# kotaro-kinoshita/yomitoku

Hardware: NVIDIA H100
Metric: pages/sec (DBNet->PARSeq OCR, synthetic 1600x1200 pages, ~200 crops/page) (higher is better)
Workload: dtype f16

## Files before the change

yomitoku_b200/csrc/gemm_tc.cu:

```cuda
#include "gemm_tc.h"

#include <cstdarg>
#include <cstdlib>
#include <cstdio>
#include <cstring>
#include <atomic>
#include <mutex>
#include <vector>

#include "ptx.cuh"

namespace ytk {

static thread_local char g_err[512] = "";
void set_error(const char* fmt, ...) {
    va_list ap;
    va_start(ap, fmt);
    vsnprintf(g_err, sizeof(g_err), fmt, ap);
    va_end(ap);
}
const char* last_error() { return g_err; }

static std::atomic<long long> g_launches{0};
void count_launch(int n) { g_launches.fetch_add(n, std::memory_order_relaxed); }
long long launch_count() { return g_launches.load(std::memory_order_relaxed); }

int pdl_launch_attr(cudaLaunchAttribute* attr) {
    static const bool on = getenv("YTK_PDL") != nullptr && getenv("YTK_NO_PDL") == nullptr;
    if (!on) return 0;
    attr[0].id = cudaLaunchAttributeProgrammaticStreamSerialization;
    attr[0].val.programmaticStreamSerializationAllowed = 1;
    return 1;
}

bool first_launch_on_device(unsigned long long* mask) {
    int d = 0;
    cudaGetDevice(&d);
    const unsigned long long bit = 1ull << (d & 63);
    if (*mask & bit) return false;
    *mask |= bit;
    return true;
}

int num_sms() {
    static int n = 0;
    if (n == 0) {
        int dev = 0;
        cudaGetDevice(&dev);
        cudaDeviceGetAttribute(&n, cudaDevAttrMultiProcessorCount, dev);
        if (n <= 0) n = 132;
    }
    return n;
}

constexpr int kBlockM = 128;
constexpr int kBlockK = 64;
constexpr int kABytes = kBlockM * kBlockK * 2;
constexpr int kThreads = 384;
constexpr int kProducerWarp = 8;
constexpr int kStagePitch = 80;
constexpr int kEpiStageBytes = 8 * 32 * kStagePitch;
constexpr int kAccPitch = 68;
constexpr int kAccBytes = 2 * 64 * kAccPitch * 4;

constexpr int kEpiBufBytes = 32 * 64;
constexpr int epi_tma_nbuf(int ) { return 2; }
constexpr int kSmemLimit = 232448;
constexpr int kSmemFixed = 1024  + 1024  + 512 ;

template <int BLOCK_N, int EPI_BYTES = kEpiStageBytes>
struct TileCfg {
    static constexpr int kBBytes = BLOCK_N * kBlockK * 2;
    static constexpr int kStageBytes = kABytes + kBBytes;
    static constexpr int kRingBudget = kSmemLimit - kSmemFixed - kAccBytes - EPI_BYTES;
    static constexpr int kStages = (kRingBudget / kStageBytes) > 8 ? 8 : (kRingBudget / kStageBytes);
    static constexpr int kRingBytes = kStages * kStageBytes;
    static constexpr int kSmemBytes = kRingBytes + kAccBytes + EPI_BYTES + kSmemFixed;
    static_assert(kStages >= 3, "K pipeline depth");
    static_assert(kSmemBytes <= kSmemLimit, "shared memory budget");
    static_assert((kRingBytes + kAccBytes) % 2048 == 0, "epilogue buffers must stay 2 KB aligned");
};

__device__ __noinline__ void copy_elems(void* dst, const void* src, int n, int esz) {
    if (esz == 4)
        for (int e = 0; e < n; ++e) reinterpret_cast<uint32_t*>(dst)[e] = reinterpret_cast<const uint32_t*>(src)[e];
    else
        for (int e = 0; e < n; ++e) reinterpret_cast<uint16_t*>(dst)[e] = reinterpret_cast<const uint16_t*>(src)[e];
}
__device__ __forceinline__ float gelu_fast(float x) {
    const float t = fminf(fabsf(x), 5.7f);
    float p = fmaf(4.278742836e-06f, t, -1.279820572e-05f);
    p = fmaf(p, t, -5.757861654e-04f);
    p = fmaf(p, t, 7.670783438e-03f);
    p = fmaf(p, t, -5.294856429e-02f);
    p = fmaf(p, t, -4.590439200e-01f);
    p = fmaf(p, t, -1.151126981e+00f);
    const float a = __fmul_rn(p, t);
    float e;
    asm("ex2.approx.ftz.f32 %0, %1;" : "=f"(e) : "f"(a));
    return fmaf(__fmul_rn(t, -0.5f), e, fmaxf(x, 0.f));
}
__device__ __forceinline__ void gelu_fast2(float& x0, float& x1) {
    x0 = gelu_fast(x0);
    x1 = gelu_fast(x1);
}

struct TileCoord {
    int img, h0, w0, n0;
};
__device__ __forceinline__ TileCoord decode_tile(const GemmArgs& a, int tile, int block_n) {
    TileCoord t;
    int m_tile = tile / a.tiles_n;
    int n_tile = tile - m_tile * a.tiles_n;
    int tw = m_tile % a.tiles_w;
    int t2 = m_tile / a.tiles_w;
    int th = t2 % a.tiles_h;
    t.img = t2 / a.tiles_h;
    t.h0 = th * (kBlockM >> a.bw_log2);
    t.w0 = tw << a.bw_log2;
    t.n0 = n_tile * block_n;
    return t;
}

template <int BLOCK_N, int RESID, int DIRECT>
using KernelCfg = TileCfg<BLOCK_N, DIRECT == 2 ? 8 * epi_tma_nbuf(RESID) * kEpiBufBytes : kEpiStageBytes>;

template <int BLOCK_N, int OUT_F32, int RESID, int MODE, int DIRECT>
__global__ void __launch_bounds__(kThreads, 1) gemm_tc_kernel(const __grid_constant__ GemmMaps maps,
                                                              const __grid_constant__ GemmArgs args) {
    using Cfg = KernelCfg<BLOCK_N, RESID, DIRECT>;
    constexpr int kEpiBytes = Cfg::kSmemBytes - Cfg::kRingBytes - kAccBytes - kSmemFixed;
    constexpr int stage_bytes = Cfg::kStageBytes;
    constexpr int nstages = Cfg::kStages;
    extern __shared__ uint8_t smem_raw[];
    const uint32_t raw_addr = smem_u32(smem_raw);
    uint8_t* smem = smem_raw + ((1024u - (raw_addr & 1023u)) & 1023u);
    const int worker = static_cast<int>(blockIdx.x);
    const int n_workers = static_cast<int>(gridDim.x);

    float* acc_smem = reinterpret_cast<float*>(smem + Cfg::kRingBytes);
    uint8_t* epi_stage = smem + Cfg::kRingBytes + kAccBytes;
    float* fin_w = reinterpret_cast<float*>(epi_stage + kEpiBytes);
    uint64_t* full_bar = reinterpret_cast<uint64_t*>(epi_stage + kEpiBytes + 1024);
    uint64_t* empty_bar = full_bar + 8;
    [[maybe_unused]] uint64_t* rbar_base = empty_bar + 8;

    const int warp = threadIdx.x >> 5;
    const int lane = threadIdx.x & 31;

    if (threadIdx.x == 0) {
        for (int i = 0; i < nstages; ++i) {
            mbar_init(&full_bar[i], 1);
            mbar_init(&empty_bar[i], 8);
        }
        if constexpr (DIRECT == 2 && RESID != 0) {
            for (int i = 0; i < 32; ++i) mbar_init(&rbar_base[i], 1);
        }
        fence_mbar_init();
        tma_prefetch_desc(&maps.a[0]);
        tma_prefetch_desc(&maps.b);
        if constexpr (DIRECT == 2) {
            tma_prefetch_desc(&maps.out);
            if constexpr (RESID != 0) {
                tma_prefetch_desc(&maps.resid);
                tma_prefetch_desc(&maps.resid_pf);
            }
        }
    }
    if constexpr (MODE == EPI_CONVT_FINAL) {
        if (threadIdx.x < 256) fin_w[threadIdx.x] = args.fin_w[threadIdx.x];
    }
    __syncthreads();
    pdl_wait();
    pdl_launch_dependents();

    const int tiles_m = args.n_img * args.tiles_h * args.tiles_w;
    const int num_kb = args.ntaps * args.kpt;
    const int total_units = tiles_m * args.tiles_n;

    if (warp >= kProducerWarp) {
        setmaxnreg_dec<40>();
        if (warp == kProducerWarp && lane == 0) {
            int stage = 0;
            uint32_t phase = 0;
            [[maybe_unused]] auto prefetch_resid = [&](int u2) {
                if (u2 >= total_units) return;
                const TileCoord c2 = decode_tile(args, u2, BLOCK_N);
                tma_prefetch_l2_4d(&maps.resid_pf, c2.n0, c2.w0, c2.h0, c2.img);
            };
            if constexpr (DIRECT == 2 && RESID != 0) {
                if (args.epi_pf) prefetch_resid(worker);
            }
            for (int u = worker; u < total_units; u += n_workers) {
                const TileCoord tc = decode_tile(args, u, BLOCK_N);
                if constexpr (DIRECT == 2 && RESID != 0) {
                    if (args.epi_pf) prefetch_resid(u + n_workers);
                }
                int tap = 0, cb = 0;
                for (int kb = 0; kb < num_kb; ++kb) {
                    mbar_wait(&empty_bar[stage], phase ^ 1u);
                    uint8_t* sa = smem + stage * stage_bytes;
                    uint8_t* sb = sa + kABytes;
                    const ConvTap tp = args.taps[tap];
                    mbar_expect_tx(&full_bar[stage], Cfg::kStageBytes);
                    tma_load_4d(sa, &maps.a[tp.map], &full_bar[stage], cb * kBlockK, tc.w0 + tp.dw, tc.h0 + tp.dh,
                                tc.img);
                    tma_load_4d(sb, &maps.b, &full_bar[stage], kb * kBlockK, tc.n0, 0, 0);
                    if (++cb == args.kpt) {
                        cb = 0;
                        ++tap;
                    }
                    if (++stage == nstages) {
                        stage = 0;
                        phase ^= 1u;
                    }
                }
            }
        }
    } else {
        setmaxnreg_inc<232>();
        const int wg = warp >> 2, wl = warp & 3;
        const int q = 2 * wg + (wl & 1);
        const int wset = wl >> 1;
        float* acc_buf = acc_smem + wg * 64 * kAccPitch;
        const float* my_acc = acc_buf + ((wl & 1) * 32 + lane) * kAccPitch;
        float acc[BLOCK_N / 2];
#pragma unroll
        for (int i = 0; i < BLOCK_N / 2; ++i) acc[i] = 0.f;
        int ring_stage = 0;
        uint32_t ring_phase = 0;
        auto mma_tile = [&]() {
            const uint32_t a_off = static_cast<uint32_t>(wg * 64 * 128);
            int prev = -1;
            for (int kb = 0; kb < num_kb; ++kb) {
                mbar_wait(&full_bar[ring_stage], ring_phase);
                const uint32_t a_addr = smem_u32(smem + ring_stage * stage_bytes);
                const uint64_t da = wgmma_desc_sw128(a_addr + a_off);
                const uint64_t db = wgmma_desc_sw128(a_addr + kABytes);
                reg_fence(acc);
                wgmma_fence();
#pragma unroll
                for (int k = 0; k < kBlockK / 16; ++k)
                    wgmma_ss<BLOCK_N>(acc, da + static_cast<uint64_t>(2 * k), db + static_cast<uint64_t>(2 * k),
                                      (kb | k) != 0 ? 1u : 0u);
                wgmma_commit();
                wgmma_wait<1>();
                reg_fence(acc);
                if (prev >= 0) {
                    __syncwarp();
                    if (lane == 0) mbar_arrive(&empty_bar[prev]);
                }
                prev = ring_stage;
                if (++ring_stage == nstages) {
                    ring_stage = 0;
                    ring_phase ^= 1u;
                }
            }
            wgmma_wait<0>();
            reg_fence(acc);
            __syncwarp();
            if (lane == 0) mbar_arrive(&empty_bar[prev]);
        };
        auto dump_slice = [&](int s) {
            named_bar_sync(1 + wg, 128);
            const int r0 = wl * 16 + (lane >> 2), c2 = (lane & 3) * 2;
#pragma unroll
            for (int j = 0; j < BLOCK_N / 8; ++j) {
                if ((j >> 3) == s) {
                    float* p = acc_buf + r0 * kAccPitch + (j & 7) * 8 + c2;
                    *reinterpret_cast<float2*>(p) = make_float2(acc[4 * j], acc[4 * j + 1]);
                    *reinterpret_cast<float2*>(p + 8 * kAccPitch) = make_float2(acc[4 * j + 2], acc[4 * j + 3]);
                }
            }
            named_bar_sync(1 + wg, 128);
        };
        auto load_chunk = [&](int c, float (&f)[32]) {
            const float4* a4 = reinterpret_cast<const float4*>(my_acc + (c & 1) * 32);
#pragma unroll
            for (int j = 0; j < 8; ++j) {
                const float4 x = a4[j];
                f[4 * j + 0] = x.x;
                f[4 * j + 1] = x.y;
                f[4 * j + 2] = x.z;
                f[4 * j + 3] = x.w;
            }
        };
        if constexpr (DIRECT == 2) {
            static_assert(MODE == EPI_NORMAL, "TMA epilogue: plain stores only");
            static_assert(RESID == 0 || (RESID == 2) == (OUT_F32 != 0), "TMA epilogue: residual and output boxes match");
            constexpr int NBUF = epi_tma_nbuf(RESID);
            constexpr int LOOK = NBUF - 1;
            constexpr int CPP = OUT_F32 ? 16 : 32;
            constexpr int NPASS = 32 / CPP;
            const int bw_mask = (1 << args.bw_log2) - 1;
            const int qw = (q * 32) & bw_mask;
            const int qh = (q * 32) >> args.bw_log2;
            uint8_t* bufs = epi_stage + warp * (NBUF * kEpiBufBytes);
            [[maybe_unused]] uint64_t* rbar = rbar_base + warp * 4;
            const int sw = args.epi_swz ? ((lane >> 1) & 3) : 0;
            const int row_off = lane * 64;
            [[maybe_unused]] int pf_u = worker, pf_c = wset, pf_p = 0, pf_g = 0;
            [[maybe_unused]] TileCoord pf_tc{};
            [[maybe_unused]] auto pf_seek = [&]() {
                while (pf_u < total_units) {
                    pf_tc = decode_tile(args, pf_u, BLOCK_N);
                    if (pf_c < BLOCK_N / 32 && pf_tc.n0 + pf_c * 32 + pf_p * CPP < args.Cout) return;
                    pf_c = wset;
                    pf_p = 0;
                    pf_u += n_workers;
                }
            };
            [[maybe_unused]] auto pf_step = [&]() {
                if (++pf_p == NPASS) {
                    pf_p = 0;
                    pf_c += 2;
                }
                pf_seek();
            };
            [[maybe_unused]] auto pf_issue = [&]() {
                const int b = pf_g % NBUF;
                mbar_expect_tx(&rbar[b], kEpiBufBytes);
                tma_load_4d(bufs + b * kEpiBufBytes, &maps.resid, &rbar[b], pf_tc.n0 + pf_c * 32 + pf_p * CPP,
                            pf_tc.w0 + qw, pf_tc.h0 + qh, pf_tc.img);
                ++pf_g;
            };
            if constexpr (RESID != 0) {
                if (lane == 0) {
                    pf_seek();
                    for (int k = 0; k < LOOK && pf_u < total_units; ++k) {
                        pf_issue();
                        pf_step();
                    }
                }
            }
            int gc = 0;
            for (int u = worker; u < total_units; u += n_workers) {
                const TileCoord tc = decode_tile(args, u, BLOCK_N);
                mma_tile();
#pragma unroll 1
                for (int c = 0; c < BLOCK_N / 32; ++c) {
                    const int col0 = tc.n0 + c * 32;
                    if ((c & 1) == 0) {
                        if (col0 >= args.Cout) break;
                        dump_slice(c >> 1);
                    }
                    if ((c & 1) != wset || col0 >= args.Cout) continue;
                    float f[32];
                    load_chunk(c, f);
                    if (args.bias != nullptr) {
                        if (col0 + 32 <= args.Cout) {
                            const float4* b4 = reinterpret_cast<const float4*>(args.bias + col0);
#pragma unroll
                            for (int j = 0; j < 8; ++j) {
                                const float4 b = __ldg(b4 + j);
                                f[4 * j + 0] += b.x;
                                f[4 * j + 1] += b.y;
                                f[4 * j + 2] += b.z;
                                f[4 * j + 3] += b.w;
                            }
                        } else {
#pragma unroll
                            for (int j = 0; j < 32; ++j) f[j] += __ldg(args.bias + min(col0 + j, args.Cout - 1));
                        }
                    }
#pragma unroll
                    for (int p = 0; p < NPASS; ++p) {
                        if (col0 + p * CPP < args.Cout) {
                            const int b = gc % NBUF;
                            uint8_t* box = bufs + b * kEpiBufBytes;
                            uint8_t* my_row = box + row_off;
                            if constexpr (RESID != 0) {
                                mbar_wait(&rbar[b], static_cast<uint32_t>(gc / NBUF) & 1u);
#pragma unroll
                                for (int j = 0; j < 4; ++j) {
                                    const uint4 r = *reinterpret_cast<const uint4*>(my_row + ((j ^ sw) << 4));
                                    if constexpr (RESID == 2) {
                                        f[p * 16 + 4 * j + 0] += __uint_as_float(r.x);
                                        f[p * 16 + 4 * j + 1] += __uint_as_float(r.y);
                                        f[p * 16 + 4 * j + 2] += __uint_as_float(r.z);
                                        f[p * 16 + 4 * j + 3] += __uint_as_float(r.w);
                                    } else {
                                        const int e = p * CPP + 8 * j;
                                        f[e + 0] += op_lo(r.x); f[e + 1] += op_hi(r.x);
                                        f[e + 2] += op_lo(r.y); f[e + 3] += op_hi(r.y);
                                        f[e + 4] += op_lo(r.z); f[e + 5] += op_hi(r.z);
                                        f[e + 6] += op_lo(r.w); f[e + 7] += op_hi(r.w);
                                    }
                                }
                            } else {
                                if (lane == 0) bulk_wait_read<NBUF - 1>();
                                __syncwarp();
                            }
                            if (args.act == ACT_RELU) {
#pragma unroll
                                for (int j = 0; j < CPP; ++j) f[p * CPP + j] = fmaxf(f[p * CPP + j], 0.f);
                            } else if (args.act == ACT_GELU) {
#pragma unroll
                                for (int j = 0; j < CPP; j += 2) gelu_fast2(f[p * CPP + j], f[p * CPP + j + 1]);
                            } else if (args.act == ACT_SIGMOID) {
#pragma unroll
                                for (int j = 0; j < CPP; ++j)
                                    f[p * CPP + j] = __fdividef(1.f, 1.f + __expf(-f[p * CPP + j]));
                            } else if (args.act == ACT_SILU) {
#pragma unroll
                                for (int j = 0; j < CPP; ++j)
                                    f[p * CPP + j] = __fdividef(f[p * CPP + j], 1.f + __expf(-f[p * CPP + j]));
                            }
#pragma unroll
                            for (int j = 0; j < 4; ++j) {
                                uint4 o;
                                if constexpr (OUT_F32) {
                                    o.x = __float_as_uint(f[p * 16 + 4 * j + 0]);
                                    o.y = __float_as_uint(f[p * 16 + 4 * j + 1]);
                                    o.z = __float_as_uint(f[p * 16 + 4 * j + 2]);
                                    o.w = __float_as_uint(f[p * 16 + 4 * j + 3]);
                                } else {
                                    const int e = p * CPP + 8 * j;
                                    o.x = pack_op(f[e + 0], f[e + 1]);
                                    o.y = pack_op(f[e + 2], f[e + 3]);
                                    o.z = pack_op(f[e + 4], f[e + 5]);
                                    o.w = pack_op(f[e + 6], f[e + 7]);
                                }
                                *reinterpret_cast<uint4*>(my_row + ((j ^ sw) << 4)) = o;
                            }
                            fence_proxy_async_smem();
                            __syncwarp();
                            if (lane == 0) {
                                tma_store_4d(&maps.out, box, col0 + p * CPP, tc.w0 + qw, tc.h0 + qh, tc.img);
                                bulk_commit();
                                if constexpr (RESID != 0) {
                                    if (pf_u < total_units) {
                                        bulk_wait_read<1>();
                                        pf_issue();
                                        pf_step();
                                    }
                                }
                            }
                            ++gc;
                        }
                    }
                }
            }
            if (lane == 0) bulk_wait_read<0>();
            __syncwarp();
        } else {
        constexpr bool kFin = (MODE == EPI_CONVT_FINAL);
        constexpr bool kWide = (OUT_F32 != 0) || (RESID == 2);
        constexpr int CPP = kWide ? 16 : 32;
        constexpr int NPASS = 32 / CPP;
        constexpr int OESZ = OUT_F32 ? 4 : 2;
        constexpr int RESZ = (RESID == 2) ? 4 : 2;
        const int row = q * 32 + lane;
        const int bw_mask = (1 << args.bw_log2) - 1;
        uint8_t* stage = epi_stage + warp * (32 * kStagePitch);
        uint8_t* my_row = stage + lane * kStagePitch;
        const int piece = lane & 3;
        for (int u = worker; u < total_units; u += n_workers) {
            const TileCoord tc = decode_tile(args, u, BLOCK_N);
            const int hh = tc.h0 + (row >> args.bw_log2);
            const int ww = tc.w0 + (row & bw_mask);
            const bool row_ok = (hh < args.Ho) && (ww < args.Wo);
            int c_h[4], c_w[4];
            bool c_ok[4];
#pragma unroll
            for (int it = 0; it < 4; ++it) {
                const int rr = q * 32 + it * 8 + (lane >> 2);
                c_h[it] = tc.h0 + (rr >> args.bw_log2);
                c_w[it] = tc.w0 + (rr & bw_mask);
                c_ok[it] = (c_h[it] < args.Ho) && (c_w[it] < args.Wo);
            }
            mma_tile();
            [[maybe_unused]] float dots[4] = {0.f, 0.f, 0.f, 0.f};
            [[maybe_unused]] float rm_m = -INFINITY, rm_s = 0.f;
            [[maybe_unused]] int rm_i = 0x7fffffff;
#pragma unroll 1
            for (int c = 0; c < BLOCK_N / 32; ++c) {
                const int col0 = tc.n0 + c * 32;
                if ((c & 1) == 0) {
                    if (col0 >= args.Cout) break;
                    dump_slice(c >> 1);
                }
                if (((kFin ? (c >> 1) : c) & 1) != wset) continue;
                if (col0 >= args.Cout) continue;
                [[maybe_unused]] uint4 dres[RESID == 2 ? 8 : 4];
                if constexpr (RESID != 0 && !kFin && DIRECT == 1) {
                    const long long pixo = (static_cast<long long>(tc.img) * args.Ho + hh) * args.Wo + ww;
                    const bool fullc = row_ok && (col0 + 32 <= args.Cout);
                    const uint4* gp = reinterpret_cast<const uint4*>(reinterpret_cast<const char*>(args.resid) +
                                                                     (pixo * args.ldr + col0) * RESZ);
#pragma unroll
                    for (int j = 0; j < (RESID == 2 ? 8 : 4); ++j) dres[j] = fullc ? gp[j] : make_uint4(0, 0, 0, 0);
                }
                [[maybe_unused]] uint4 rres[NPASS][4];
                if constexpr (RESID != 0 && !kFin && DIRECT == 0) {
                    constexpr int per16r = 16 / RESZ;
                    int ocol_r = col0, sub_r = 0;
                    if constexpr (MODE == EPI_SHUFFLE2X) {
                        const int cq = args.Cout >> 2;
                        sub_r = col0 / cq;
                        ocol_r = col0 - sub_r * cq;
                    }
#pragma unroll
                    for (int p = 0; p < NPASS; ++p) {
                        const int validr = min(CPP, args.Cout - (col0 + p * CPP));
                        const int e0 = piece * per16r;
#pragma unroll
                        for (int it = 0; it < 4; ++it) {
                            rres[p][it] = make_uint4(0, 0, 0, 0);
                            if (c_ok[it] && e0 + per16r <= validr) {
                                const long long pixr =
                                    (static_cast<long long>(tc.img) * args.Ho + c_h[it]) * args.Wo + c_w[it];
                                const char* gp = reinterpret_cast<const char*>(args.resid) +
                                                 (pixr * args.ldr + ocol_r + p * CPP + e0) * RESZ;
                                rres[p][it] = *reinterpret_cast<const uint4*>(gp);
                            }
                        }
                    }
                }
                float f[32];
                load_chunk(c, f);
                if (args.bias != nullptr) {
                    if (col0 + 32 <= args.Cout) {
                        const float4* b4 = reinterpret_cast<const float4*>(args.bias + col0);
#pragma unroll
                        for (int j = 0; j < 8; ++j) {
                            const float4 b = __ldg(b4 + j);
                            f[4 * j + 0] += b.x;
                            f[4 * j + 1] += b.y;
                            f[4 * j + 2] += b.z;
                            f[4 * j + 3] += b.w;
                        }
                    } else {
#pragma unroll
                        for (int j = 0; j < 32; ++j) f[j] += __ldg(args.bias + min(col0 + j, args.Cout - 1));
                    }
                }
                if constexpr (MODE == EPI_ROWMAX) {
                    const int nvalid = min(32, args.Cout - col0);
                    float cm = -INFINITY;
                    int ci = 0x7fffffff;
#pragma unroll
                    for (int j = 0; j < 32; ++j) {
                        const float v = j < nvalid ? f[j] : -INFINITY;
                        f[j] = v;
                        if (v > cm) {
                            cm = v;
                            ci = col0 + j;
                        }
                    }
                    float cs = 0.f;
                    if (args.act != ACT_RELU) {
#pragma unroll
                        for (int j = 0; j < 32; ++j) cs += __expf(f[j] - cm);
                    }
                    if (cm > rm_m) {
                        rm_s = rm_s * __expf(rm_m - cm) + cs;
                        rm_m = cm;
                        rm_i = ci;
                    } else {
                        rm_s += cs * __expf(cm - rm_m);
                    }
                } else if constexpr (kFin) {
                    const int chan0 = (c & 1) * 32;
#pragma unroll
                    for (int j = 0; j < 32; ++j) {
                        const float x = fmaxf(f[j], 0.f);
#pragma unroll
                        for (int k = 0; k < 4; ++k) dots[k] += x * fin_w[k * 64 + chan0 + j];
                    }
                    if (c & 1) {
                        if (row_ok) {
                            const int sub = c >> 1;
                            const long long oy = 2LL * (2 * hh + (sub >> 1)), ox = 2LL * (2 * ww + (sub & 1));
                            float* op = reinterpret_cast<float*>(args.out) +
                                        (static_cast<long long>(tc.img) * (4 * args.Ho) + oy) * (4LL * args.Wo) + ox;
                            float2 r0, r1;
                            r0.x = 1.f / (1.f + __expf(-(dots[0] + args.fin_b)));
                            r0.y = 1.f / (1.f + __expf(-(dots[1] + args.fin_b)));
                            r1.x = 1.f / (1.f + __expf(-(dots[2] + args.fin_b)));
                            r1.y = 1.f / (1.f + __expf(-(dots[3] + args.fin_b)));
                            *reinterpret_cast<float2*>(op) = r0;
                            *reinterpret_cast<float2*>(op + 4LL * args.Wo) = r1;
                        }
                        dots[0] = dots[1] = dots[2] = dots[3] = 0.f;
                    }
                } else if constexpr (DIRECT == 1) {
                    int ocol = col0, sub = 0;
                    long long opix = (static_cast<long long>(tc.img) * args.Ho + hh) * args.Wo + ww;
                    if constexpr (MODE == EPI_SHUFFLE2X) {
                        const int cq = args.Cout >> 2;
                        sub = col0 / cq;
                        ocol = col0 - sub * cq;
                        opix = (static_cast<long long>(tc.img) * (2 * args.Ho) + (2 * hh + (sub >> 1))) * (2LL * args.Wo) +
// ... 121 lines not shown
                                        const float4 r = rp[j];
                                        f[p * 16 + 4 * j + 0] += r.x;
                                        f[p * 16 + 4 * j + 1] += r.y;
                                        f[p * 16 + 4 * j + 2] += r.z;
                                        f[p * 16 + 4 * j + 3] += r.w;
                                    }
                                } else {
                                    const uint4* rp = reinterpret_cast<const uint4*>(my_row);
#pragma unroll
                                    for (int j = 0; j < CPP / 8; ++j) {
                                        const uint4 r = rp[j];
                                        const int b = p * CPP + 8 * j;
                                        f[b + 0] += op_lo(r.x); f[b + 1] += op_hi(r.x);
                                        f[b + 2] += op_lo(r.y); f[b + 3] += op_hi(r.y);
                                        f[b + 4] += op_lo(r.z); f[b + 5] += op_hi(r.z);
                                        f[b + 6] += op_lo(r.w); f[b + 7] += op_hi(r.w);
                                    }
                                }
                                __syncwarp();
                            }
                            if (args.act == ACT_RELU) {
#pragma unroll
                                for (int j = 0; j < CPP; ++j) f[p * CPP + j] = fmaxf(f[p * CPP + j], 0.f);
                            } else if (args.act == ACT_GELU) {
#pragma unroll
                                for (int j = 0; j < CPP; j += 2) gelu_fast2(f[p * CPP + j], f[p * CPP + j + 1]);
                            } else if (args.act == ACT_SIGMOID) {
#pragma unroll
                                for (int j = 0; j < CPP; ++j)
                                    f[p * CPP + j] = __fdividef(1.f, 1.f + __expf(-f[p * CPP + j]));
                            } else if (args.act == ACT_SILU) {
#pragma unroll
                                for (int j = 0; j < CPP; ++j)
                                    f[p * CPP + j] = __fdividef(f[p * CPP + j], 1.f + __expf(-f[p * CPP + j]));
                            }
                            if constexpr (OUT_F32) {
                                float4* wp = reinterpret_cast<float4*>(my_row);
#pragma unroll
                                for (int j = 0; j < 4; ++j) {
                                    float4 o;
                                    o.x = f[p * 16 + 4 * j + 0];
                                    o.y = f[p * 16 + 4 * j + 1];
                                    o.z = f[p * 16 + 4 * j + 2];
                                    o.w = f[p * 16 + 4 * j + 3];
                                    wp[j] = o;
                                }
                            } else {
                                uint4* wp = reinterpret_cast<uint4*>(my_row);
#pragma unroll
                                for (int j = 0; j < CPP / 8; ++j) {
                                    const int b = p * CPP + 8 * j;
                                    uint4 o;
                                    o.x = pack_op(f[b + 0], f[b + 1]);
                                    o.y = pack_op(f[b + 2], f[b + 3]);
                                    o.z = pack_op(f[b + 4], f[b + 5]);
                                    o.w = pack_op(f[b + 6], f[b + 7]);
                                    wp[j] = o;
                                }
                            }
                            __syncwarp();
                            {
                                constexpr int per16 = 16 / OESZ;
                                constexpr int row_bytes = CPP * OESZ;
                                const int e0 = piece * per16;
                                if (piece * 16 < row_bytes && e0 < valid) {
#pragma unroll
                                    for (int it = 0; it < 4; ++it) {
                                        if (!c_ok[it]) continue;
                                        const int rr = it * 8 + (lane >> 2);
                                        const uint8_t* sp = stage + rr * kStagePitch + piece * 16;
                                        char* gp = reinterpret_cast<char*>(args.out) +
                                                   (c_pix[it] * args.ldc + pc0 + e0) * OESZ;
                                        if (e0 + per16 <= valid) {
                                            *reinterpret_cast<uint4*>(gp) = *reinterpret_cast<const uint4*>(sp);
                                        } else {
                                            copy_elems(gp, sp, valid - e0, OESZ);
                                        }
                                    }
                                }
                            }
                            __syncwarp();
                        }
                    }
                }
            }
            if constexpr (MODE == EPI_ROWMAX) {
                if (row_ok) {
                    const long long pixo = (static_cast<long long>(tc.img) * args.Ho + hh) * args.Wo + ww;
                    float4 o;
                    o.x = rm_m;
                    o.y = rm_s;
                    o.z = __int_as_float(rm_i);
                    o.w = 0.f;
                    reinterpret_cast<float4*>(args.out)[pixo * args.ldc + (tc.n0 / BLOCK_N) * 2 + wset] = o;
                }
            }
        }
        }
    }
}

typedef CUresult (*EncodeTiledFn)(CUtensorMap*, CUtensorMapDataType, cuuint32_t, void*, const cuuint64_t*,
                                  const cuuint64_t*, const cuuint32_t*, const cuuint32_t*, CUtensorMapInterleave,
                                  CUtensorMapSwizzle, CUtensorMapL2promotion, CUtensorMapFloatOOBfill);

static EncodeTiledFn get_encode_fn() {
    static EncodeTiledFn fn = nullptr;
    static std::once_flag once;
    std::call_once(once, []() {
        void* p = nullptr;
        cudaDriverEntryPointQueryResult qres;
        cudaError_t e = cudaGetDriverEntryPoint("cuTensorMapEncodeTiled", &p, cudaEnableDefault, &qres);
        if (e == cudaSuccess && qres == cudaDriverEntryPointSuccess) fn = reinterpret_cast<EncodeTiledFn>(p);
    });
    return fn;
}

int make_tmap_op_4d(CUtensorMap* m, const void* base, const uint64_t dims[4], const uint64_t strides_b[3],
                      const uint32_t box[4]) {
    EncodeTiledFn fn = get_encode_fn();
    if (!fn) {
        set_error("cuTensorMapEncodeTiled entry point unavailable (no CUDA driver?)");
        return 1;
    }
    cuuint64_t gd[4] = {dims[0], dims[1], dims[2], dims[3]};
    cuuint64_t gs[3] = {strides_b[0], strides_b[1], strides_b[2]};
    cuuint32_t bx[4] = {box[0], box[1], box[2], box[3]};
    cuuint32_t es[4] = {1, 1, 1, 1};
    CUresult r = fn(m, kOpFmt ? CU_TENSOR_MAP_DATA_TYPE_BFLOAT16 : CU_TENSOR_MAP_DATA_TYPE_FLOAT16, 4, const_cast<void*>(base), gd, gs, bx, es,
                    CU_TENSOR_MAP_INTERLEAVE_NONE, CU_TENSOR_MAP_SWIZZLE_128B, CU_TENSOR_MAP_L2_PROMOTION_L2_256B,
                    CU_TENSOR_MAP_FLOAT_OOB_FILL_NONE);
    if (r != CUDA_SUCCESS) {
        set_error("cuTensorMapEncodeTiled failed (%d): dims=%llu,%llu,%llu,%llu strides=%llu,%llu,%llu box=%u,%u,%u,%u "
                  "base=%p",
                  (int)r, (unsigned long long)dims[0], (unsigned long long)dims[1], (unsigned long long)dims[2],
                  (unsigned long long)dims[3], (unsigned long long)strides_b[0], (unsigned long long)strides_b[1],
                  (unsigned long long)strides_b[2], box[0], box[1], box[2], box[3], base);
        return 1;
    }
    return 0;
}

static int make_tmap_epi(CUtensorMap* m, const void* base, int f32, const GemmArgs& a, int Cout, long long ld, int swz,
                         int tile_cols = 0) {
    EncodeTiledFn fn = get_encode_fn();
    if (!fn) {
        set_error("cuTensorMapEncodeTiled entry point unavailable (no CUDA driver?)");
        return 1;
    }
    const uint64_t es = f32 ? 4 : 2;
    const int bw = 1 << a.bw_log2;
    cuuint64_t gd[4] = {(cuuint64_t)Cout, (cuuint64_t)a.Wo, (cuuint64_t)a.Ho, (cuuint64_t)a.n_img};
    cuuint64_t gs[3] = {(cuuint64_t)ld * es, (cuuint64_t)ld * es * a.Wo, (cuuint64_t)ld * es * a.Wo * a.Ho};
    cuuint32_t bx[4] = {(cuuint32_t)(64 / es), (cuuint32_t)(bw < 32 ? bw : 32), (cuuint32_t)(bw < 32 ? 32 / bw : 1), 1};
    if (tile_cols > 0) {
        bx[0] = (cuuint32_t)tile_cols;
        bx[1] = (cuuint32_t)bw;
        bx[2] = (cuuint32_t)(128 / bw);
        swz = 0;
    }
    static const bool l2_256 = getenv("YTK_EPI_L2P") != nullptr && getenv("YTK_EPI_L2P")[0] == '2';
    cuuint32_t est[4] = {1, 1, 1, 1};
    const CUtensorMapDataType dt = f32 ? CU_TENSOR_MAP_DATA_TYPE_FLOAT32
                                       : (kOpFmt ? CU_TENSOR_MAP_DATA_TYPE_BFLOAT16 : CU_TENSOR_MAP_DATA_TYPE_FLOAT16);
    CUresult r = fn(m, dt, 4, const_cast<void*>(base), gd, gs, bx, est, CU_TENSOR_MAP_INTERLEAVE_NONE,
                    swz ? CU_TENSOR_MAP_SWIZZLE_64B : CU_TENSOR_MAP_SWIZZLE_NONE,
                    l2_256 ? CU_TENSOR_MAP_L2_PROMOTION_L2_256B : CU_TENSOR_MAP_L2_PROMOTION_L2_128B,
                    CU_TENSOR_MAP_FLOAT_OOB_FILL_NONE);
    if (r != CUDA_SUCCESS) {
        set_error("cuTensorMapEncodeTiled (epilogue box) failed (%d): dims=%llu,%llu,%llu,%llu ld=%lld f32=%d base=%p",
                  (int)r, (unsigned long long)gd[0], (unsigned long long)gd[1], (unsigned long long)gd[2],
                  (unsigned long long)gd[3], ld, f32, base);
        return 1;
    }
    return 0;
}

static int epi_mode_env() {
    static int mode = -1;
    if (mode < 0) {
        const char* e = getenv("YTK_EPI");
        mode = (e && e[0] == 's') ? 0 : 2;
    }
    return mode;
}

static int pick_block_n(int Cout) {
    if (Cout <= 64) return 64;
    if (Cout <= 128) return 128;
    if (Cout % 256 == 0 || Cout > 512) return 256;
    if (Cout % 128 == 0) return 128;
    return 256;
}

static int pick_bw_log2(int Ho, int Wo) {
    int best = 7;
    long long best_cost = -1;
    for (int l = 3; l <= 7; ++l) {
        int bw = 1 << l, bh = 128 >> l;
        long long cost = (long long)((Wo + bw - 1) / bw) * ((Ho + bh - 1) / bh);
        if (best_cost < 0 || cost < best_cost || (cost == best_cost && l > best)) {
            best_cost = cost;
            best = l;
        }
    }
    return best;
}

static int finish_plan(GemmPlan* plan, const void* w_packed, int Ktot, int Cout, const Epilogue& e) {
    GemmArgs& a = plan->args;
    plan->block_n = pick_block_n(Cout);
    static const bool no_shrink = getenv("YTK_NO_SHRINK") != nullptr;
    static const bool no_wave_model = getenv("YTK_WAVE_MODEL") == nullptr;
    if (e.mode != EPI_CONVT_FINAL && !no_shrink) {
        const int m_tiles = a.n_img * a.tiles_h * a.tiles_w;
        const int sms = num_sms();
        auto tiles_at = [&](int bn) { return (long long)m_tiles * ((Cout + bn - 1) / bn); };
        if (no_wave_model || (tiles_at(plan->block_n) + sms - 1) / sms > 6) {
            while (plan->block_n > 64 && tiles_at(plan->block_n) < sms) plan->block_n >>= 1;
        } else {
            int best = plan->block_n;
            double best_cost = 1e30;
            for (int bn = plan->block_n; bn >= 64; bn >>= 1) {
                const double w = bn == 256 ? 1.9 : bn == 128 ? 1.0 : 0.56;
                const double cost = (double)((tiles_at(bn) + sms - 1) / sms) * w;
                if (cost < best_cost - 1e-9) {
                    best_cost = cost;
                    best = bn;
                }
            }
            plan->block_n = best;
        }
    }
    a.tiles_n = (Cout + plan->block_n - 1) / plan->block_n;
    a.Cout = Cout;
    a.bias = e.bias;
    a.resid = e.resid;
    a.resid_f32 = e.resid_f32;
    a.ldr = e.ldr;
    a.out = e.out;
    a.out_f32 = e.out_f32;
    a.ldc = e.ldc;
    a.act = e.act;
    a.mode = e.mode;
    a.fin_w = e.fin_w;
    a.fin_b = e.fin_b;
    if (e.out == nullptr) {
        set_error("gemm plan: null output");
        return 1;
    }
    if (e.mode == EPI_ROWMAX) {
        if (e.resid != nullptr) {
            set_error("gemm plan: ROWMAX takes no residual");
            return 1;
        }
        a.out_f32 = 1;
        a.ldc = 2LL * a.tiles_n;
    } else if (e.mode == EPI_CONVT_FINAL) {
        if (Cout != 256 || e.fin_w == nullptr || !e.out_f32) {
            set_error("gemm plan: CONVT_FINAL needs Cout=256, fp32 output and the final conv weights");
            return 1;
        }
    } else if ((e.out_f32 ? (e.ldc % 4) : (e.ldc % 8)) != 0) {
        set_error("gemm plan: ldc=%lld must keep rows 16-byte aligned", e.ldc);
        return 1;
    }
    if (e.resid && ((e.resid_f32 ? (e.ldr % 4) : (e.ldr % 8)) != 0)) {
        set_error("gemm plan: ldr=%lld must keep rows 16-byte aligned", e.ldr);
        return 1;
    }
    if (e.mode == EPI_SHUFFLE2X && ((Cout % 4) != 0 || ((Cout / 4) % 32) != 0)) {
        set_error("gemm plan: SHUFFLE2X needs Cout/4 to be a multiple of 32 (Cout=%d)", Cout);
        return 1;
    }
    const int tiles = a.n_img * a.tiles_h * a.tiles_w * a.tiles_n;
    a.epi_tma = 0;
    a.epi_swz = 0;
    a.epi_pf = 0;
    if (epi_mode_env() == 2 && e.mode == EPI_NORMAL && (e.resid == nullptr || (e.resid_f32 != 0) == (e.out_f32 != 0)) &&
        ((long long)Cout * (e.out_f32 ? 4 : 2)) % 16 == 0 &&
        (reinterpret_cast<uintptr_t>(e.out) & 15) == 0 && (reinterpret_cast<uintptr_t>(e.resid) & 15) == 0) {
        static const bool no_swz = getenv("YTK_EPI_SWZ") != nullptr && getenv("YTK_EPI_SWZ")[0] == '0';
        static const bool no_pf = !(getenv("YTK_EPI_PF") != nullptr && getenv("YTK_EPI_PF")[0] == '1');
        a.epi_tma = 1;
        a.epi_swz = no_swz ? 0 : 1;
        if (make_tmap_epi(&plan->maps.out, e.out, e.out_f32, a, Cout, e.ldc, a.epi_swz)) return 1;
        if (e.resid != nullptr) {
            if (make_tmap_epi(&plan->maps.resid, e.resid, e.resid_f32, a, Cout, e.ldr, a.epi_swz)) return 1;
            if (make_tmap_epi(&plan->maps.resid_pf, e.resid, e.resid_f32, a, Cout, e.ldr, 0, plan->block_n)) return 1;
            a.epi_pf = no_pf ? 0 : 1;
        } else {
            plan->maps.resid = plan->maps.out;
            plan->maps.resid_pf = plan->maps.out;
        }
    }
    uint64_t dims[4] = {(uint64_t)Ktot, (uint64_t)Cout, 1, 1};
    uint64_t strides[3] = {(uint64_t)Ktot * 2, (uint64_t)Ktot * 2 * Cout, (uint64_t)Ktot * 2 * Cout};
    uint32_t box[4] = {(uint32_t)kBlockK, (uint32_t)plan->block_n, 1, 1};
    if (make_tmap_op_4d(&plan->maps.b, w_packed, dims, strides, box)) return 1;
    plan->grid = tiles < num_sms() ? tiles : num_sms();
    if (plan->grid < 1) plan->grid = 1;
    return 0;
}

int conv_plan_create(GemmPlan* plan, const void* in, const ConvGeom& g, const void* w_packed, const Epilogue& e) {
    memset(plan, 0, sizeof(*plan));
    GemmArgs& a = plan->args;
    if (g.Cin % kBlockK != 0) {
        set_error("conv plan: Cin=%d must be a multiple of %d", g.Cin, kBlockK);
        return 1;
    }
    if (g.stride != 1 && g.stride != 2) {
        set_error("conv plan: stride %d unsupported", g.stride);
        return 1;
    }
    if (g.kh * g.kw > kMaxTaps) {
        set_error("conv plan: %dx%d filter exceeds %d taps", g.kh, g.kw, kMaxTaps);
        return 1;
    }
// ... 317 lines not shown
```

Baseline: 43.97.

## Write TMA epilogue straight from MMA fragments via stmatrix, dropping smem accumulator staging

Reworks the TMA-store epilogue so each warp takes its 16-row slice of the accumulator fragments from registers and writes them into 128B-swizzled 16x128B boxes with stmatrix. Residual tiles are read back with ldmatrix. This removes the float accumulator dump to shared memory (the acc buffer is zero-sized for this path), and the freed space goes to four TMA buffers per warp and possibly a deeper K ring. The box shape and swizzle mode of the tensor maps change to match. The new fragment-to-address mapping and swizzle math carry correctness risk, and the epilogue now relies on per-warp fragment ownership.

```diff
diff --git a/yomitoku_b200/csrc/gemm_tc.cu b/yomitoku_b200/csrc/gemm_tc.cu
--- a/yomitoku_b200/csrc/gemm_tc.cu
+++ b/yomitoku_b200/csrc/gemm_tc.cu
@@ -63,23 +63,36 @@
 constexpr int kAccPitch = 68;
 constexpr int kAccBytes = 2 * 64 * kAccPitch * 4;
 
-constexpr int kEpiBufBytes = 32 * 64;
-constexpr int epi_tma_nbuf(int ) { return 2; }
+constexpr int kEpiBufBytes = 16 * 128;
+constexpr int kEpiTmaBufs = 4;
 constexpr int kSmemLimit = 232448;
 constexpr int kSmemFixed = 1024  + 1024  + 512 ;
 
-template <int BLOCK_N, int EPI_BYTES = kEpiStageBytes>
+template <int BLOCK_N, int EPI_BYTES = kEpiStageBytes, int ACC_BYTES = kAccBytes>
 struct TileCfg {
     static constexpr int kBBytes = BLOCK_N * kBlockK * 2;
     static constexpr int kStageBytes = kABytes + kBBytes;
-    static constexpr int kRingBudget = kSmemLimit - kSmemFixed - kAccBytes - EPI_BYTES;
+    static constexpr int kAccB = ACC_BYTES;
+    static constexpr int kRingBudget = kSmemLimit - kSmemFixed - ACC_BYTES - EPI_BYTES;
     static constexpr int kStages = (kRingBudget / kStageBytes) > 8 ? 8 : (kRingBudget / kStageBytes);
     static constexpr int kRingBytes = kStages * kStageBytes;
-    static constexpr int kSmemBytes = kRingBytes + kAccBytes + EPI_BYTES + kSmemFixed;
+    static constexpr int kSmemBytes = kRingBytes + ACC_BYTES + EPI_BYTES + kSmemFixed;
     static_assert(kStages >= 3, "K pipeline depth");
     static_assert(kSmemBytes <= kSmemLimit, "shared memory budget");
-    static_assert((kRingBytes + kAccBytes) % 2048 == 0, "epilogue buffers must stay 2 KB aligned");
+    static_assert((kRingBytes + ACC_BYTES) % 2048 == 0, "epilogue buffers must stay 2 KB aligned");
 };
+
+__device__ __forceinline__ void ldsm_x4(uint32_t addr, uint32_t& r0, uint32_t& r1, uint32_t& r2, uint32_t& r3) {
+    asm volatile("ldmatrix.sync.aligned.m8n8.x4.shared.b16 {%0, %1, %2, %3}, [%4];"
+                 : "=r"(r0), "=r"(r1), "=r"(r2), "=r"(r3)
+                 : "r"(addr)
+                 : "memory");
+}
+__device__ __forceinline__ void stsm_x4(uint32_t addr, uint32_t r0, uint32_t r1, uint32_t r2, uint32_t r3) {
+    asm volatile("stmatrix.sync.aligned.m8n8.x4.shared.b16 [%0], {%1, %2, %3, %4};" ::"r"(addr), "r"(r0), "r"(r1),
+                 "r"(r2), "r"(r3)
+                 : "memory");
+}
 
 __device__ __noinline__ void copy_elems(void* dst, const void* src, int n, int esz) {
     if (esz == 4)
@@ -123,13 +136,14 @@
 }
 
 template <int BLOCK_N, int RESID, int DIRECT>
-using KernelCfg = TileCfg<BLOCK_N, DIRECT == 2 ? 8 * epi_tma_nbuf(RESID) * kEpiBufBytes : kEpiStageBytes>;
+using KernelCfg = TileCfg<BLOCK_N, DIRECT == 2 ? 8 * kEpiTmaBufs * kEpiBufBytes : kEpiStageBytes,
+                          DIRECT == 2 ? 0 : kAccBytes>;
 
 template <int BLOCK_N, int OUT_F32, int RESID, int MODE, int DIRECT>
 __global__ void __launch_bounds__(kThreads, 1) gemm_tc_kernel(const __grid_constant__ GemmMaps maps,
                                                               const __grid_constant__ GemmArgs args) {
     using Cfg = KernelCfg<BLOCK_N, RESID, DIRECT>;
-    constexpr int kEpiBytes = Cfg::kSmemBytes - Cfg::kRingBytes - kAccBytes - kSmemFixed;
+    constexpr int kEpiBytes = Cfg::kSmemBytes - Cfg::kRingBytes - Cfg::kAccB - kSmemFixed;
     constexpr int stage_bytes = Cfg::kStageBytes;
     constexpr int nstages = Cfg::kStages;
     extern __shared__ uint8_t smem_raw[];
@@ -139,7 +153,7 @@
     const int n_workers = static_cast<int>(gridDim.x);
 
     float* acc_smem = reinterpret_cast<float*>(smem + Cfg::kRingBytes);
-    uint8_t* epi_stage = smem + Cfg::kRingBytes + kAccBytes;
+    uint8_t* epi_stage = smem + Cfg::kRingBytes + Cfg::kAccB;
     float* fin_w = reinterpret_cast<float*>(epi_stage + kEpiBytes);
     uint64_t* full_bar = reinterpret_cast<uint64_t*>(epi_stage + kEpiBytes + 1024);
     uint64_t* empty_bar = full_bar + 8;
@@ -288,40 +302,42 @@
         if constexpr (DIRECT == 2) {
             static_assert(MODE == EPI_NORMAL, "TMA epilogue: plain stores only");
             static_assert(RESID == 0 || (RESID == 2) == (OUT_F32 != 0), "TMA epilogue: residual and output boxes match");
-            constexpr int NBUF = epi_tma_nbuf(RESID);
+            constexpr int NBUF = kEpiTmaBufs;
+            static_assert(NBUF <= 4, "residual barriers: 4 per warp");
             constexpr int LOOK = NBUF - 1;
-            constexpr int CPP = OUT_F32 ? 16 : 32;
-            constexpr int NPASS = 32 / CPP;
+            constexpr int CPB = OUT_F32 ? 32 : 64;
+            constexpr int JPB = CPB / 8;
+            constexpr int NPASS = BLOCK_N / CPB;
+            const int tr0 = warp * 16;
             const int bw_mask = (1 << args.bw_log2) - 1;
-            const int qw = (q * 32) & bw_mask;
-            const int qh = (q * 32) >> args.bw_log2;
+            const int qw = tr0 & bw_mask;
+            const int qh = tr0 >> args.bw_log2;
             uint8_t* bufs = epi_stage + warp * (NBUF * kEpiBufBytes);
             [[maybe_unused]] uint64_t* rbar = rbar_base + warp * 4;
-            const int sw = args.epi_swz ? ((lane >> 1) & 3) : 0;
-            const int row_off = lane * 64;
-            [[maybe_unused]] int pf_u = worker, pf_c = wset, pf_p = 0, pf_g = 0;
+            const int swz = args.epi_swz ? 7 : 0;
+            const int fr = lane >> 2;
+            const int fc = (lane & 3) * 2;
+            const int f32_sub = (lane >> 1) & 1, f32_byte = (lane & 1) * 8;
+            const int mrow = ((lane >> 3) & 1) * 8 + (lane & 7), mchunk = lane >> 4;
+            [[maybe_unused]] int pf_u = worker, pf_p = 0, pf_g = 0;
             [[maybe_unused]] TileCoord pf_tc{};
             [[maybe_unused]] auto pf_seek = [&]() {
                 while (pf_u < total_units) {
                     pf_tc = decode_tile(args, pf_u, BLOCK_N);
-                    if (pf_c < BLOCK_N / 32 && pf_tc.n0 + pf_c * 32 + pf_p * CPP < args.Cout) return;
-                    pf_c = wset;
+                    if (pf_p < NPASS && pf_tc.n0 + pf_p * CPB < args.Cout) return;
                     pf_p = 0;
                     pf_u += n_workers;
                 }
             };
             [[maybe_unused]] auto pf_step = [&]() {
-                if (++pf_p == NPASS) {
-                    pf_p = 0;
-                    pf_c += 2;
-                }
+                ++pf_p;
                 pf_seek();
             };
             [[maybe_unused]] auto pf_issue = [&]() {
                 const int b = pf_g % NBUF;
                 mbar_expect_tx(&rbar[b], kEpiBufBytes);
-                tma_load_4d(bufs + b * kEpiBufBytes, &maps.resid, &rbar[b], pf_tc.n0 + pf_c * 32 + pf_p * CPP,
-                            pf_tc.w0 + qw, pf_tc.h0 + qh, pf_tc.img);
+                tma_load_4d(bufs + b * kEpiBufBytes, &maps.resid, &rbar[b], pf_tc.n0 + pf_p * CPB, pf_tc.w0 + qw,
+                            pf_tc.h0 + qh, pf_tc.img);
                 ++pf_g;
             };
             if constexpr (RESID != 0) {
@@ -337,108 +353,98 @@
             for (int u = worker; u < total_units; u += n_workers) {
                 const TileCoord tc = decode_tile(args, u, BLOCK_N);
                 mma_tile();
-#pragma unroll 1
-                for (int c = 0; c < BLOCK_N / 32; ++c) {
-                    const int col0 = tc.n0 + c * 32;
-                    if ((c & 1) == 0) {
-                        if (col0 >= args.Cout) break;
-                        dump_slice(c >> 1);
-                    }
-                    if ((c & 1) != wset || col0 >= args.Cout) continue;
-                    float f[32];
-                    load_chunk(c, f);
+#pragma unroll
+                for (int p = 0; p < NPASS; ++p) {
+                    const int col0 = tc.n0 + p * CPB;
+                    if (col0 >= args.Cout) break;
+                    const int b = gc % NBUF;
+                    uint8_t* box = bufs + b * kEpiBufBytes;
+                    const uint32_t box_s = smem_u32(box);
+                    float v[4 * JPB];
+#pragma unroll
+                    for (int i = 0; i < 4 * JPB; ++i) v[i] = acc[4 * JPB * p + i];
                     if (args.bias != nullptr) {
-                        if (col0 + 32 <= args.Cout) {
-                            const float4* b4 = reinterpret_cast<const float4*>(args.bias + col0);
-#pragma unroll
-                            for (int j = 0; j < 8; ++j) {
-                                const float4 b = __ldg(b4 + j);
-                                f[4 * j + 0] += b.x;
-                                f[4 * j + 1] += b.y;
-                                f[4 * j + 2] += b.z;
-                                f[4 * j + 3] += b.w;
+#pragma unroll
+                        for (int jj = 0; jj < JPB; ++jj) {
+                            const int col = col0 + 8 * jj + fc;
+                            const float2 bb = col < args.Cout ? __ldg(reinterpret_cast<const float2*>(args.bias + col))
+                                                              : make_float2(0.f, 0.f);
+                            v[4 * jj + 0] += bb.x;
+                            v[4 * jj + 1] += bb.y;
+                            v[4 * jj + 2] += bb.x;
+                            v[4 * jj + 3] += bb.y;
+                        }
+                    }
+                    if constexpr (RESID != 0) {
+                        mbar_wait(&rbar[b], static_cast<uint32_t>(gc / NBUF) & 1u);
+                        if constexpr (RESID == 2) {
+#pragma unroll
+                            for (int jj = 0; jj < JPB; ++jj) {
+                                const uint8_t* rp = box + fr * 128 + (((2 * jj + f32_sub) ^ (fr & swz)) << 4) + f32_byte;
+                                const float2 r0 = *reinterpret_cast<const float2*>(rp);
+                                const float2 r1 = *reinterpret_cast<const float2*>(rp + 1024);
+                                v[4 * jj + 0] += r0.x;
+                                v[4 * jj + 1] += r0.y;
+                                v[4 * jj + 2] += r1.x;
+                                v[4 * jj + 3] += r1.y;
                             }
                         } else {
 #pragma unroll
-                            for (int j = 0; j < 32; ++j) f[j] += __ldg(args.bias + min(col0 + j, args.Cout - 1));
+                            for (int t = 0; t < JPB / 2; ++t) {
+                                uint32_t r0, r1, r2, r3;
+                                ldsm_x4(box_s + mrow * 128 + (((2 * t + mchunk) ^ (mrow & swz)) << 4), r0, r1, r2, r3);
+                                v[8 * t + 0] += op_lo(r0); v[8 * t + 1] += op_hi(r0);
+                                v[8 * t + 2] += op_lo(r1); v[8 * t + 3] += op_hi(r1);
+                                v[8 * t + 4] += op_lo(r2); v[8 * t + 5] += op_hi(r2);
+                                v[8 * t + 6] += op_lo(r3); v[8 * t + 7] += op_hi(r3);
+                            }
                         }
-                    }
-#pragma unroll
-                    for (int p = 0; p < NPASS; ++p) {
-                        if (col0 + p * CPP < args.Cout) {
-                            const int b = gc % NBUF;
-                            uint8_t* box = bufs + b * kEpiBufBytes;
-                            uint8_t* my_row = box + row_off;
-                            if constexpr (RESID != 0) {
-                                mbar_wait(&rbar[b], static_cast<uint32_t>(gc / NBUF) & 1u);
-#pragma unroll
-                                for (int j = 0; j < 4; ++j) {
-                                    const uint4 r = *reinterpret_cast<const uint4*>(my_row + ((j ^ sw) << 4));
-                                    if constexpr (RESID == 2) {
-                                        f[p * 16 + 4 * j + 0] += __uint_as_float(r.x);
-                                        f[p * 16 + 4 * j + 1] += __uint_as_float(r.y);
-                                        f[p * 16 + 4 * j + 2] += __uint_as_float(r.z);
-                                        f[p * 16 + 4 * j + 3] += __uint_as_float(r.w);
-                                    } else {
-                                        const int e = p * CPP + 8 * j;
-                                        f[e + 0] += op_lo(r.x); f[e + 1] += op_hi(r.x);
-                                        f[e + 2] += op_lo(r.y); f[e + 3] += op_hi(r.y);
-                                        f[e + 4] += op_lo(r.z); f[e + 5] += op_hi(r.z);
-                                        f[e + 6] += op_lo(r.w); f[e + 7] += op_hi(r.w);
-                                    }
-                                }
-                            } else {
-                                if (lane == 0) bulk_wait_read<NBUF - 1>();
-                                __syncwarp();
+                        __syncwarp();
+                    } else {
+                        if (lane == 0) bulk_wait_read<NBUF - 1>();
+                        __syncwarp();
+                    }
+                    if (args.act == ACT_RELU) {
+#pragma unroll
+                        for (int j = 0; j < 4 * JPB; ++j) v[j] = fmaxf(v[j], 0.f);
+                    } else if (args.act == ACT_GELU) {
+#pragma unroll
+                        for (int j = 0; j < 4 * JPB; j += 2) gelu_fast2(v[j], v[j + 1]);
+                    } else if (args.act == ACT_SIGMOID) {
+#pragma unroll
+                        for (int j = 0; j < 4 * JPB; ++j) v[j] = __fdividef(1.f, 1.f + __expf(-v[j]));
+                    } else if (args.act == ACT_SILU) {
+#pragma unroll
+                        for (int j = 0; j < 4 * JPB; ++j) v[j] = __fdividef(v[j], 1.f + __expf(-v[j]));
+                    }
+                    if constexpr (OUT_F32) {
+#pragma unroll
+                        for (int jj = 0; jj < JPB; ++jj) {
+                            uint8_t* wp = box + fr * 128 + (((2 * jj + f32_sub) ^ (fr & swz)) << 4) + f32_byte;
+                            *reinterpret_cast<float2*>(wp) = make_float2(v[4 * jj + 0], v[4 * jj + 1]);
+                            *reinterpret_cast<float2*>(wp + 1024) = make_float2(v[4 * jj + 2], v[4 * jj + 3]);
+                        }
+                    } else {
+#pragma unroll
+                        for (int t = 0; t < JPB / 2; ++t)
+                            stsm_x4(box_s + mrow * 128 + (((2 * t + mchunk) ^ (mrow & swz)) << 4),
+                                    pack_op(v[8 * t + 0], v[8 * t + 1]), pack_op(v[8 * t + 2], v[8 * t + 3]),
+                                    pack_op(v[8 * t + 4], v[8 * t + 5]), pack_op(v[8 * t + 6], v[8 * t + 7]));
+                    }
+                    fence_proxy_async_smem();
+                    __syncwarp();
+                    if (lane == 0) {
+                        tma_store_4d(&maps.out, box, col0, tc.w0 + qw, tc.h0 + qh, tc.img);
+                        bulk_commit();
+                        if constexpr (RESID != 0) {
+                            if (pf_u < total_units) {
+                                bulk_wait_read<1>();
+                                pf_issue();
+                                pf_step();
                             }
-                            if (args.act == ACT_RELU) {
-#pragma unroll
-                                for (int j = 0; j < CPP; ++j) f[p * CPP + j] = fmaxf(f[p * CPP + j], 0.f);
-                            } else if (args.act == ACT_GELU) {
-#pragma unroll
-                                for (int j = 0; j < CPP; j += 2) gelu_fast2(f[p * CPP + j], f[p * CPP + j + 1]);
-                            } else if (args.act == ACT_SIGMOID) {
-#pragma unroll
-                                for (int j = 0; j < CPP; ++j)
-                                    f[p * CPP + j] = __fdividef(1.f, 1.f + __expf(-f[p * CPP + j]));
-                            } else if (args.act == ACT_SILU) {
-#pragma unroll
-                                for (int j = 0; j < CPP; ++j)
-                                    f[p * CPP + j] = __fdividef(f[p * CPP + j], 1.f + __expf(-f[p * CPP + j]));
-                            }
-#pragma unroll
-                            for (int j = 0; j < 4; ++j) {
-                                uint4 o;
-                                if constexpr (OUT_F32) {
-                                    o.x = __float_as_uint(f[p * 16 + 4 * j + 0]);
-                                    o.y = __float_as_uint(f[p * 16 + 4 * j + 1]);
-                                    o.z = __float_as_uint(f[p * 16 + 4 * j + 2]);
-                                    o.w = __float_as_uint(f[p * 16 + 4 * j + 3]);
-                                } else {
-                                    const int e = p * CPP + 8 * j;
-                                    o.x = pack_op(f[e + 0], f[e + 1]);
-                                    o.y = pack_op(f[e + 2], f[e + 3]);
-                                    o.z = pack_op(f[e + 4], f[e + 5]);
-                                    o.w = pack_op(f[e + 6], f[e + 7]);
-                                }
-                                *reinterpret_cast<uint4*>(my_row + ((j ^ sw) << 4)) = o;
-                            }
-                            fence_proxy_async_smem();
-                            __syncwarp();
-                            if (lane == 0) {
-                                tma_store_4d(&maps.out, box, col0 + p * CPP, tc.w0 + qw, tc.h0 + qh, tc.img);
-                                bulk_commit();
-                                if constexpr (RESID != 0) {
-                                    if (pf_u < total_units) {
-                                        bulk_wait_read<1>();
-                                        pf_issue();
-                                        pf_step();
-                                    }
-                                }
-                            }
-                            ++gc;
                         }
                     }
+                    ++gc;
                 }
             }
             if (lane == 0) bulk_wait_read<0>();
@@ -866,7 +872,7 @@
     const int bw = 1 << a.bw_log2;
     cuuint64_t gd[4] = {(cuuint64_t)Cout, (cuuint64_t)a.Wo, (cuuint64_t)a.Ho, (cuuint64_t)a.n_img};
     cuuint64_t gs[3] = {(cuuint64_t)ld * es, (cuuint64_t)ld * es * a.Wo, (cuuint64_t)ld * es * a.Wo * a.Ho};
-    cuuint32_t bx[4] = {(cuuint32_t)(64 / es), (cuuint32_t)(bw < 32 ? bw : 32), (cuuint32_t)(bw < 32 ? 32 / bw : 1), 1};
+    cuuint32_t bx[4] = {(cuuint32_t)(128 / es), (cuuint32_t)(bw < 16 ? bw : 16), (cuuint32_t)(bw < 16 ? 16 / bw : 1), 1};
     if (tile_cols > 0) {
         bx[0] = (cuuint32_t)tile_cols;
         bx[1] = (cuuint32_t)bw;
@@ -878,7 +884,7 @@
     const CUtensorMapDataType dt = f32 ? CU_TENSOR_MAP_DATA_TYPE_FLOAT32
                                        : (kOpFmt ? CU_TENSOR_MAP_DATA_TYPE_BFLOAT16 : CU_TENSOR_MAP_DATA_TYPE_FLOAT16);
     CUresult r = fn(m, dt, 4, const_cast<void*>(base), gd, gs, bx, est, CU_TENSOR_MAP_INTERLEAVE_NONE,
-                    swz ? CU_TENSOR_MAP_SWIZZLE_64B : CU_TENSOR_MAP_SWIZZLE_NONE,
+                    swz ? CU_TENSOR_MAP_SWIZZLE_128B : CU_TENSOR_MAP_SWIZZLE_NONE,
                     l2_256 ? CU_TENSOR_MAP_L2_PROMOTION_L2_256B : CU_TENSOR_MAP_L2_PROMOTION_L2_128B,
                     CU_TENSOR_MAP_FLOAT_OOB_FILL_NONE);
     if (r != CUDA_SUCCESS) {
```

Result: faster. 46.38, median of 6 (+5.5%).
